# antoyang/FrozenBiLM

Hardware: AMD Instinct MI355X
Metric: video-text samples/sec (MLM fwd+bwd) DeBERTa-XL+adapters (higher is better)
Workload: dtype bf16; 1 GPU; DeBERTa-v2-XLarge(24L)+adapters ds8/8, B=32/GPU, T=10x1024, L=256 (S=266), MLM fwd+bwd+allreduce+clip+Adam, dropout 0.1 live, seeded random weights; global_batch=32, seq_len=266, parallelism=dp1, dead_layer23_encoder_pass=skipped (output unused, SURVEY fact 6); FLOPs still counted

## Files before the change

### frozenbilm_amd/csrc/attn_fwd.hip

```cpp
#include "attn_common.h"
#include "../../include/fbl.h"

namespace {
using namespace attn;

struct AttnArgs {
  const bf16* q; const bf16* k; const bf16* v; const bf16* pk; const bf16* pq;
  long ldq, ldk, ldp;
  long ldv;
  const int16_t* relidx;
  const int32_t* mask;
  const int32_t* klen;
  const int32_t* border;
  float scale, p_drop;
  uint64_t seed; const uint64_t* seed_dev;
  bf16* ctx;
  long ldo;
  float* lse;
  int B, S, Sp, nh, span2;
  int lin;
  int dbg;
  const int32_t* row0;
  bf16* psave;
  float* msave;
};
#ifdef FBL_DEBUG_SWITCHES
#define ATTN_DBG(bit) (a.dbg & (bit))
#else
#define ATTN_DBG(bit) 0
#endif

constexpr int LTW = 100;
constexpr int SM_KS = 0;
constexpr int SM_VS = SM_KS + 8192;
constexpr int SM_T1 = SM_VS + 8192;
constexpr int SM_T2 = SM_T1 + 64 * LTW * 2;
constexpr int SM_KM = SM_T2 + 64 * LTW * 2;
constexpr int SM_QS = SM_KM + 256;
constexpr int SM_IDX = SM_QS + 8192;
__host__ __device__ constexpr int sm_total(int Sp) { return SM_IDX + 2 * Sp * 2; }

struct TileRegs {
  bf16x8 k[2], v[2];
  int km;
};

template <int OCC, bool PF, bool PACKED = false, bool SAVEP = false>
__global__ __launch_bounds__(256, OCC) void attn_fwd_kernel(AttnArgs a) {
  extern __shared__ __attribute__((aligned(16))) char smem[];
  const int tid = threadIdx.x, lane = tid & 63;
  const int w = __builtin_amdgcn_readfirstlane(tid >> 6);
  const int c = lane & 15, g = lane >> 4;
  const int S = a.S, Sp = a.Sp;
  const WgCoord wc = wg_coord((S + 63) / 64, a.nh, a.B, a.border);
  const int i0 = wc.x * 64, h = wc.h, b = wc.b;
  const int i = i0 + w * 16 + c;
  const int ic = min(i, S - 1);

  int16_t* idx = (int16_t*)(smem + SM_IDX);
  float* kms = (float*)(smem + SM_KM);
  f16* T1 = (f16*)(smem + SM_T1);
  f16* T2 = (f16*)(smem + SM_T2);

  const int kl = a.klen ? min(a.klen[b], S) : S;
  const int nkt = (i0 < kl) ? (kl + 63) / 64 : 0;
  const long rb = PACKED ? (long)a.row0[b] : (long)b * S;
  const int lim = PACKED ? min(a.row0[b + 1] - a.row0[b], S) : S;
  if (nkt > 0) load_idx_padded(idx, a.relidx, S, Sp, tid, 256);

  const bool qvalid = i < S && a.mask[(long)b * S + ic] != 0;

  float m_run = -INFINITY, l_run = 0.f;
  f32x4 o[4];
#pragma unroll
  for (int dt = 0; dt < 4; ++dt) o[dt] = (f32x4){0.f, 0.f, 0.f, 0.f};

  const DropKey dk = attn_drop_key(a.p_drop > 0.f ? fbl_seed(a.seed, a.seed_dev) : 0, b * a.nh + h, a.p_drop);
  const float k2 = a.scale * LOG2E;
  const int tq = Sp - 1;
  const int izero = a.relidx[S - 1];
  const bf16* pkh = a.pk + h * 64 + g * 8;
  const bf16* pqh = a.pq + h * 64 + g * 8;
  const int my_t0 = (0x5243 >> (w * 4)) & 15, my_t1 = (0x1670 >> (w * 4)) & 15;

  const int srow = tid >> 3, sch = tid & 7;
  const int fb0 = c * 128 + ((g ^ (c & 7)) << 4), fb1 = fb0 ^ 64;
  const int sb = srow * 128 + ((sch ^ (srow & 7)) << 4);
  auto load_tile = [&](int jt, TileRegs& R) {
    const int j0 = jt * 64;
#pragma unroll
    for (int t = 0; t < 2; ++t) {
      const int row = srow + t * 32;
      const int j = min(j0 + row, lim - 1);
      R.k[t] = *(const bf16x8*)(a.k + (rb + j) * a.ldk + h * 64 + sch * 8);
      R.v[t] = *(const bf16x8*)(a.v + (rb + j) * a.ldv + h * 64 + sch * 8);
    }
    R.km = a.mask[(long)b * S + min(j0 + lane, S - 1)];
  };
  auto store_tile = [&](const TileRegs& R, int j0) {
#pragma unroll
    for (int t = 0; t < 2; ++t) {
      *(bf16x8*)(smem + SM_KS + sb + t * 4096) = R.k[t];
      *(bf16x8*)(smem + SM_VS + sb + t * 4096) = R.v[t];
    }
    if (tid < 64) kms[tid] = (j0 + tid < S && R.km != 0) ? 1.f : 0.f;
  };

  TileRegs R;
  if (PF && nkt > 0) load_tile(0, R);
  if (nkt > 0) {
#pragma unroll
    for (int t = 0; t < 2; ++t) {
      const int row = srow + t * 32;
      *(bf16x8*)(smem + SM_QS + sb + t * 4096) = *(const bf16x8*)(a.q + (rb + min(i0 + row, lim - 1)) * a.ldq + h * 64 + sch * 8);
    }
    __syncthreads();
  }
  for (int jt = 0; jt < nkt; ++jt) {
    const int j0 = jt * 64;
    const bool band = !ATTN_DBG(32) && max(abs(i0 - (j0 + 63)), abs(i0 + 63 - j0)) < a.lin;
    int r_lo, t0q[4], t0k[4];
    if (band) {
      r_lo = izero + i0 - (j0 + 63);
#pragma unroll
      for (int x = 0; x < 4; ++x) { t0q[x] = x; t0k[x] = 3 - x; }
    } else {
      r_lo = __builtin_amdgcn_readfirstlane((int)idx[i0 - (j0 + 63) + tq]);
#pragma unroll
      for (int x = 0; x < 4; ++x) {
        t0q[x] = (__builtin_amdgcn_readfirstlane((int)idx[i0 + x * 16 - (j0 + 63) + tq]) - r_lo) >> 4;
        t0k[x] = (__builtin_amdgcn_readfirstlane((int)idx[i0 - (j0 + x * 16 + 15) + tq]) - r_lo) >> 4;
      }
    }
    const int ntile = band ? 5 : 6;
    bf16x8 apk[2][2], apq[2][2];
    if (!ATTN_DBG(2)) {
#pragma unroll
      for (int u = 0; u < 2; ++u) {
        const long ro = (long)min(r_lo + (u ? my_t1 : my_t0) * 16 + c, a.span2 - 1) * a.ldp;
        apk[u][0] = *(const bf16x8*)(pkh + ro);
        apk[u][1] = *(const bf16x8*)(pkh + ro + 32);
        apq[u][0] = *(const bf16x8*)(pqh + ro);
        apq[u][1] = *(const bf16x8*)(pqh + ro + 32);
      }
    }
    if (!PF) load_tile(jt, R);
    store_tile(R, j0);
    __syncthreads();

    f32x4 sacc[4];
    const bf16x8 qf[2] = {*(const bf16x8*)(smem + SM_QS + w * 2048 + fb0), *(const bf16x8*)(smem + SM_QS + w * 2048 + fb1)};
#pragma unroll
    for (int nt = 0; nt < 4; ++nt) {
      f32x4 acc = (f32x4){0.f, 0.f, 0.f, 0.f};
      acc = __builtin_amdgcn_mfma_f32_16x16x32_bf16(*(const bf16x8*)(smem + SM_KS + nt * 2048 + fb0), qf[0], acc, 0, 0, 0);
      acc = __builtin_amdgcn_mfma_f32_16x16x32_bf16(*(const bf16x8*)(smem + SM_KS + nt * 2048 + fb1), qf[1], acc, 0, 0, 0);
      sacc[nt] = acc;
    }
    if (!ATTN_DBG(2)) {
      const f16 ninf = (f16)(-INFINITY);
      f16* t1s = T1 + c * LTW + g * 4;
      f16* t2s = T2 + c * LTW + g * 4;
      auto pair1 = [&](const bf16x8& a0, const bf16x8& a1, int x, int rel) {
        f32x4 acc = (f32x4){0.f, 0.f, 0.f, 0.f};
        acc = __builtin_amdgcn_mfma_f32_16x16x32_bf16(a0, *(const bf16x8*)(smem + SM_QS + x * 2048 + fb0), acc, 0, 0, 0);
        acc = __builtin_amdgcn_mfma_f32_16x16x32_bf16(a1, *(const bf16x8*)(smem + SM_QS + x * 2048 + fb1), acc, 0, 0, 0);
        *(f16x4*)(t1s + x * 16 * LTW + rel * 16) = to_f16x4(acc);
      };
      auto pair2 = [&](const bf16x8& a0, const bf16x8& a1, int x, int rel) {
        f32x4 acc = (f32x4){0.f, 0.f, 0.f, 0.f};
        acc = __builtin_amdgcn_mfma_f32_16x16x32_bf16(a0, *(const bf16x8*)(smem + SM_KS + x * 2048 + fb0), acc, 0, 0, 0);
        acc = __builtin_amdgcn_mfma_f32_16x16x32_bf16(a1, *(const bf16x8*)(smem + SM_KS + x * 2048 + fb1), acc, 0, 0, 0);
        const f16x4 tv = to_f16x4(acc);
        *(f16x4*)(t2s + x * 16 * LTW + rel * 16) = kms[x * 16 + c] != 0.f ? tv : (f16x4){ninf, ninf, ninf, ninf};
      };
      {
#pragma unroll
        for (int u = 0; u < 2; ++u) {
          const int t = u ? my_t1 : my_t0;
#pragma unroll
          for (int x = 0; x < 4; ++x) {
            const int rel1 = t - t0q[x];
            if (rel1 >= 0 && rel1 < ntile) pair1(apk[u][0], apk[u][1], x, rel1);
            const int rel2 = t - t0k[x];
            if (rel2 >= 0 && rel2 < ntile) pair2(apq[u][0], apq[u][1], x, rel2);
          }
        }
      }
    }
    __syncthreads();
    if (PF) load_tile(min(jt + 1, nkt - 1), R);

    float p[16];
    float mx = -INFINITY;
    if (ATTN_DBG(1)) {
#pragma unroll
      for (int e = 0; e < 16; ++e) { p[e] = sacc[e >> 2][e & 3]; mx = fmaxf(mx, p[e]); }
    } else if (band) {
      const f16* t1p = T1 + (w * 16 + c) * LTW + c + 63 - g * 4;
      const f16* t2p = T2 + g * 4 * LTW + w * 16 + c + 15 - g * 4;
#pragma unroll
      for (int nt = 0; nt < 4; ++nt)
#pragma unroll
        for (int r = 0; r < 4; ++r) {
          const float s = sacc[nt][r] + (float)t1p[-(nt * 16 + r)] + (float)t2p[(nt * 16 + r) * LTW - r];
          p[nt * 4 + r] = s;
          mx = fmaxf(mx, s);
        }
    } else {
      const int16_t* ib = idx + (i - j0 - g * 4 + tq - 63);
      int sbw = r_lo;
#pragma unroll
      for (int x = 0; x < 4; ++x) sbw = (w == x) ? r_lo + 16 * t0q[x] : sbw;
      const f16* t1row = T1 + (w * 16 + c) * LTW - sbw;
      const f16* t2g = T2 + g * 4 * LTW - r_lo;
#pragma unroll
      for (int nt = 0; nt < 4; ++nt) {
        const f16* t2n = t2g - 16 * t0k[nt];
#pragma unroll
        for (int r = 0; r < 4; ++r) {
          const int wi = ib[63 - nt * 16 - r];
          const float s = sacc[nt][r] + (float)t1row[wi] + (float)t2n[(nt * 16 + r) * LTW + wi];
          p[nt * 4 + r] = s;
          mx = fmaxf(mx, s);
        }
      }
    }
    mx = fmaxf(mx, __shfl_xor(mx, 16, 64));
    mx = fmaxf(mx, __shfl_xor(mx, 32, 64));
    const float m_new = fmaxf(m_run, mx);
    float alpha = 1.f, psum = 0.f;
    if (!(m_new > -INFINITY)) {
#pragma unroll
      for (int e = 0; e < 16; ++e) p[e] = 0.f;
    } else {
      alpha = __builtin_amdgcn_exp2f((m_run - m_new) * k2);
      const float mk = -m_new * k2;
#pragma unroll
      for (int e = 0; e < 16; ++e) {
        p[e] = __builtin_amdgcn_exp2f(fmaf(p[e], k2, mk));
        psum += p[e];
      }
    }
    psum += __shfl_xor(psum, 16, 64);
    psum += __shfl_xor(psum, 32, 64);
    l_run = l_run * alpha + psum;
    m_run = m_new;
#pragma unroll
    for (int dt = 0; dt < 4; ++dt) o[dt] *= alpha;
    float kf[16];
#pragma unroll
    for (int e = 0; e < 16; ++e) kf[e] = 1.f;
    if (a.p_drop > 0.f && !ATTN_DBG(8)) {
#pragma unroll
      for (int nt = 0; nt < 4; ++nt)
#pragma unroll
        for (int bb = 0; bb < 2; ++bb) {
          uint32_t x, y;
          attn_drop_block(dk, i >> 1, (j0 + nt * 16 + g * 4 + bb * 2) >> 1, Sp >> 1, &x, &y);
          kf[nt * 4 + bb * 2] = attn_drop_keep(dk, x, y, i & 1, 0);
          kf[nt * 4 + bb * 2 + 1] = attn_drop_keep(dk, x, y, i & 1, 1);
        }
    }
    if constexpr (SAVEP) {
      bf16* pp = a.psave + (((long)b * a.nh + h) * Sp + i) * Sp + j0 + g * 4;
#pragma unroll
      for (int nt = 0; nt < 4; ++nt) {
        bf16x4 v4;
#pragma unroll
        for (int r = 0; r < 4; ++r) v4[r] = f2bf(kf[nt * 4 + r] == 0.f ? -p[nt * 4 + r] : p[nt * 4 + r]);
        *(bf16x4*)(pp + nt * 16) = v4;
      }
      if (g == 0 && i < S) a.msave[(((long)b * a.nh + h) * (Sp >> 6) + jt) * S + i] = m_new * k2;
    }
#pragma unroll
    for (int e = 0; e < 16; ++e) p[e] *= kf[e];
    if (!ATTN_DBG(4))
#pragma unroll
    for (int kk = 0; kk < 2; ++kk) {
      bf16x8 pf;
#pragma unroll
      for (int e = 0; e < 4; ++e) {
        pf[e] = f2bf(p[(2 * kk) * 4 + e]);
        pf[4 + e] = f2bf(p[(2 * kk + 1) * 4 + e]);
      }
#pragma unroll
      for (int dt = 0; dt < 4; ++dt) {
        const int r = g * 4 + (c >> 2);
        const int ch = dt * 2 + ((c >> 1) & 1), sub = (c & 1) * 8;
        const char* vb = smem + SM_VS + r * 128 + ((ch ^ (r & 7)) << 4) + sub;
        union { tr16x4 h[2]; bf16x8 v; } u;
        u.h[0] = lds_tr16((const bf16*)(vb + kk * 4096));
        u.h[1] = lds_tr16((const bf16*)(vb + kk * 4096 + 2048));
        o[dt] = __builtin_amdgcn_mfma_f32_16x16x32_bf16(u.v, pf, o[dt], 0, 0, 0);
      }
    }
    __syncthreads();
  }

  const float inv_l = (qvalid && l_run > 0.f) ? 1.f / l_run : 0.f;
  if (i < S) {
    if (i < lim) {
      bf16* op = a.ctx + (rb + i) * a.ldo + h * 64 + g * 4;
#pragma unroll
      for (int dt = 0; dt < 4; ++dt) {
        f32x4 v = o[dt] * inv_l;
        if (inv_l == 0.f) v = (f32x4){0.f, 0.f, 0.f, 0.f};
        *(bf16x4*)(op + dt * 16) = (bf16x4){f2bf(v[0]), f2bf(v[1]), f2bf(v[2]), f2bf(v[3])};
      }
    }
    if (g == 0 && a.lse)
      a.lse[((long)b * a.nh + h) * S + i] = (qvalid && l_run > 0.f) ? m_run * a.scale + __logf(l_run) : INFINITY;
  }
}

__global__ __launch_bounds__(128) void attn_probs_kernel(const bf16* q, const bf16* k, long ldq, const bf16* pk, const bf16* pq,
                                                         long ldp, const int16_t* relidx, const int32_t* mask, const float* lse,
                                                         float scale, float* probs, int B, int S, int nh) {
  __shared__ float qs[64];
  const int i = blockIdx.x % S, h = (blockIdx.x / S) % nh, b = blockIdx.x / (S * nh);
  const long row = (long)b * S + i;
  if (threadIdx.x < 64) qs[threadIdx.x] = bf2f(q[row * ldq + h * 64 + threadIdx.x]);
  __syncthreads();
  const bool qvalid = mask[row] != 0;
  const float l = lse[((long)b * nh + h) * S + i];
  float* out = probs + (((long)b * nh + h) * S + i) * S;
  for (int j = threadIdx.x; j < S; j += blockDim.x) {
    float p = 0.f;
    if (qvalid && mask[(long)b * S + j] != 0) {
      const int r = relidx[i - j + S - 1];
      const bf16* kj = k + ((long)b * S + j) * ldq + h * 64;
      const bf16* pkr = pk + (long)r * ldp + h * 64;
      const bf16* pqr = pq + (long)r * ldp + h * 64;
      float s = 0.f;
#pragma unroll 8
      for (int d = 0; d < 64; ++d) {
        const float kd = bf2f(kj[d]);
        s += qs[d] * (kd + bf2f(pkr[d])) + kd * bf2f(pqr[d]);
      }
      p = __expf(s * scale - l);
    }
    out[j] = p;
  }
}

}

extern "C" int fbl_disent_attn_probs(const void* q, const void* k, int64_t ldq, const void* pk, const void* pq, int64_t ldp,
                                     const int16_t* relidx, const int32_t* mask, const float* lse, float scale,
                                     float* probs, int B, int S, int nh, void* stream) {
  if (S < 1 || S > 512) return FBL_ERR_SHAPE;
  if (!q || !k || !pk || !pq || !relidx || !mask || !lse || !probs) return FBL_ERR_ARG;
  if (B <= 0 || nh <= 0) return 0;
  hipLaunchKernelGGL(attn_probs_kernel, dim3((unsigned)(B * nh * S)), dim3(128), 0, (hipStream_t)stream, (const bf16*)q,
                     (const bf16*)k, (long)ldq, (const bf16*)pk, (const bf16*)pq, (long)ldp, relidx, mask, lse, scale, probs, B, S,
                     nh);
  FBL_CHECK_LAUNCH();
  return 0;
}

extern "C" int fbl_disent_attn_fwd(const void* q, int64_t ldq, const void* k, int64_t ldk, const void* v, int64_t ldv,
                                   const void* pk, const void* pq, int64_t ldp,
                                   const int16_t* relidx, const int32_t* mask, const int32_t* klen,
                                   const int32_t* border, float scale, float p_drop, uint64_t seed,
                                   const uint64_t* seed_dev, void* ctx, int64_t ldo, float* lse, int B, int S, int Sp, int nh, int span2,
                                   int lin_span, const int32_t* row0, void* psave, float* msave, void* stream) {
  if (S < 1 || S > 512 || Sp < S || Sp % 64) return FBL_ERR_SHAPE;
  if ((ldq % 8) || (ldk % 8) || (ldv % 8) || (ldp % 8) || (ldo % 4)) return FBL_ERR_ALIGN;
  if (lin_span < 0 || 2 * lin_span > span2) return FBL_ERR_ARG;
  if (row0 && !klen) return FBL_ERR_ARG;
  if ((psave != nullptr) != (msave != nullptr) || (psave && !lse)) return FBL_ERR_ARG;
  if (B <= 0 || nh <= 0) return 0;
  AttnArgs a{(const bf16*)q, (const bf16*)k, (const bf16*)v, (const bf16*)pk, (const bf16*)pq, ldq, ldk, ldp, ldv, relidx, mask, klen, border, scale, p_drop, seed, seed_dev, (bf16*)ctx, ldo, lse, B, S, Sp, nh, span2, lin_span, 0, row0,
             (bf16*)psave, msave};
  static const int dbg = FBL_ENV_INT("FBL_ATTN_DBG", 0);
  a.dbg = dbg;
  attn_debug_init();
  const int smem_bytes = sm_total(Sp);
  static int attr_bytes = 0;
  if (smem_bytes > attr_bytes) {
    const void* fns[] = {(const void*)attn_fwd_kernel<3, true>, (const void*)attn_fwd_kernel<3, true, true>,
                         (const void*)attn_fwd_kernel<3, true, false, true>, (const void*)attn_fwd_kernel<3, true, true, true>,
#ifdef FBL_DEBUG_SWITCHES
                         (const void*)attn_fwd_kernel<3, false>, (const void*)attn_fwd_kernel<3, false, true>,
                         (const void*)attn_fwd_kernel<3, false, false, true>, (const void*)attn_fwd_kernel<3, false, true, true>,
#endif
    };
    for (const void* fn : fns) {
      hipError_t e = hipFuncSetAttribute(fn, hipFuncAttributeMaxDynamicSharedMemorySize, smem_bytes);
      if (e != hipSuccess) return (int)e;
    }
    attr_bytes = smem_bytes;
  }
  dim3 grid((unsigned)((S + 63) / 64) * nh * B);
#define FBL_FWD_LAUNCH(PF_)                                                                                             \
  do {                                                                                                                  \
    if (row0 && psave)                                                                                                  \
      hipLaunchKernelGGL((attn_fwd_kernel<3, PF_, true, true>), grid, dim3(256), smem_bytes, (hipStream_t)stream, a);   \
    else if (row0)                                                                                                      \
      hipLaunchKernelGGL((attn_fwd_kernel<3, PF_, true>), grid, dim3(256), smem_bytes, (hipStream_t)stream, a);         \
    else if (psave)                                                                                                     \
      hipLaunchKernelGGL((attn_fwd_kernel<3, PF_, false, true>), grid, dim3(256), smem_bytes, (hipStream_t)stream, a);  \
    else                                                                                                                \
      hipLaunchKernelGGL((attn_fwd_kernel<3, PF_>), grid, dim3(256), smem_bytes, (hipStream_t)stream, a);               \
  } while (0)
#ifdef FBL_DEBUG_SWITCHES
  static const int pf = FBL_ENV_INT("FBL_ATTN_PF", 1);
  if (!pf) FBL_FWD_LAUNCH(false);
  else
#endif
    FBL_FWD_LAUNCH(true);
#undef FBL_FWD_LAUNCH
  FBL_CHECK_LAUNCH();
  return 0;
}
```

Before: 787.9 samples/s.

## Use buffer loads and prefetch position fragments one tile ahead in attention forward

Global loads for Q, K, V, positional K/Q, mask and relidx in the disentangled attention forward kernel now go through buffer resource descriptors with 32-bit offsets instead of 64-bit pointer arithmetic. The apk/apq positional fragments for the next key tile are issued right after the next K/V tile prefetch, so their latency overlaps the current tile's softmax and PV work. The prologue loads of relidx, Q and the first fragments are hoisted ahead of the LDS stores, and workgroups with no key tiles now exit early. Host checks reject leading dimensions that would overflow the 32-bit buffer offsets, and register pressure rises from holding the prefetched fragments.

```diff
diff --git a/frozenbilm_amd/csrc/attn_fwd.hip b/frozenbilm_amd/csrc/attn_fwd.hip
--- a/frozenbilm_amd/csrc/attn_fwd.hip
+++ b/frozenbilm_amd/csrc/attn_fwd.hip
@@ -45,6 +45,17 @@
   int km;
 };
 
+typedef __attribute__((ext_vector_type(2))) unsigned int u32x2;
+__device__ __forceinline__ int buf_ld4(__amdgpu_buffer_rsrc_t r, uint32_t voff, uint32_t soff) {
+  return (int)__builtin_amdgcn_raw_buffer_load_b32(r, voff, soff, 0);
+}
+__device__ __forceinline__ int16_t buf_ld2(__amdgpu_buffer_rsrc_t r, uint32_t voff, uint32_t soff) {
+  return (int16_t)__builtin_amdgcn_raw_buffer_load_b16(r, voff, soff, 0);
+}
+__device__ __forceinline__ void buf_st8(__amdgpu_buffer_rsrc_t r, uint32_t voff, uint32_t soff, bf16x4 v) {
+  __builtin_amdgcn_raw_buffer_store_b64(__builtin_bit_cast(u32x2, v), r, voff, soff, 0);
+}
+
 template <int OCC, bool PF, bool PACKED = false, bool SAVEP = false>
 __global__ __launch_bounds__(256, OCC) void attn_fwd_kernel(AttnArgs a) {
   extern __shared__ __attribute__((aligned(16))) char smem[];
@@ -66,36 +77,40 @@
   const int nkt = (i0 < kl) ? (kl + 63) / 64 : 0;
   const long rb = PACKED ? (long)a.row0[b] : (long)b * S;
   const int lim = PACKED ? min(a.row0[b + 1] - a.row0[b], S) : S;
-  if (nkt > 0) load_idx_padded(idx, a.relidx, S, Sp, tid, 256);
-
-  const bool qvalid = i < S && a.mask[(long)b * S + ic] != 0;
-
-  float m_run = -INFINITY, l_run = 0.f;
-  f32x4 o[4];
-#pragma unroll
-  for (int dt = 0; dt < 4; ++dt) o[dt] = (f32x4){0.f, 0.f, 0.f, 0.f};
-
-  const DropKey dk = attn_drop_key(a.p_drop > 0.f ? fbl_seed(a.seed, a.seed_dev) : 0, b * a.nh + h, a.p_drop);
+  if (nkt == 0) {
+    if (i < S) {
+      if (i < lim) {
+        bf16* op = a.ctx + (rb + i) * a.ldo + h * 64 + g * 4;
+#pragma unroll
+        for (int dt = 0; dt < 4; ++dt) *(bf16x4*)(op + dt * 16) = (bf16x4){f2bf(0.f), f2bf(0.f), f2bf(0.f), f2bf(0.f)};
+      }
+      if (g == 0 && a.lse) a.lse[((long)b * a.nh + h) * S + i] = INFINITY;
+    }
+    return;
+  }
+
   const float k2 = a.scale * LOG2E;
   const int tq = Sp - 1;
-  const int izero = a.relidx[S - 1];
-  const bf16* pkh = a.pk + h * 64 + g * 8;
-  const bf16* pqh = a.pq + h * 64 + g * 8;
   const int my_t0 = (0x5243 >> (w * 4)) & 15, my_t1 = (0x1670 >> (w * 4)) & 15;
 
   const int srow = tid >> 3, sch = tid & 7;
   const int fb0 = c * 128 + ((g ^ (c & 7)) << 4), fb1 = fb0 ^ 64;
   const int sb = srow * 128 + ((sch ^ (srow & 7)) << 4);
+
+  const __amdgpu_buffer_rsrc_t rq = buf_rsrc(a.q + rb * a.ldq + h * 64), rk = buf_rsrc(a.k + rb * a.ldk + h * 64),
+                               rv = buf_rsrc(a.v + rb * a.ldv + h * 64), rpk = buf_rsrc(a.pk + h * 64),
+                               rpq = buf_rsrc(a.pq + h * 64), rmask = buf_rsrc(a.mask + (long)b * S),
+                               ridx = buf_rsrc(a.relidx);
+  const uint32_t ldq2 = (uint32_t)a.ldq * 2, ldk2 = (uint32_t)a.ldk * 2, ldv2 = (uint32_t)a.ldv * 2, ldp2 = (uint32_t)a.ldp * 2;
   auto load_tile = [&](int jt, TileRegs& R) {
     const int j0 = jt * 64;
 #pragma unroll
     for (int t = 0; t < 2; ++t) {
-      const int row = srow + t * 32;
-      const int j = min(j0 + row, lim - 1);
-      R.k[t] = *(const bf16x8*)(a.k + (rb + j) * a.ldk + h * 64 + sch * 8);
-      R.v[t] = *(const bf16x8*)(a.v + (rb + j) * a.ldv + h * 64 + sch * 8);
-    }
-    R.km = a.mask[(long)b * S + min(j0 + lane, S - 1)];
+      const uint32_t j = (uint32_t)min(j0 + srow + t * 32, lim - 1);
+      R.k[t] = buf_ld16(rk, j * ldk2 + sch * 16, 0);
+      R.v[t] = buf_ld16(rv, j * ldv2 + sch * 16, 0);
+    }
+    R.km = buf_ld4(rmask, (uint32_t)min(j0 + lane, S - 1) * 4, 0);
   };
   auto store_tile = [&](const TileRegs& R, int j0) {
 #pragma unroll
@@ -105,27 +120,62 @@
     }
     if (tid < 64) kms[tid] = (j0 + tid < S && R.km != 0) ? 1.f : 0.f;
   };
-
+  auto in_band = [&](int j0) { return !ATTN_DBG(32) && max(abs(i0 - (j0 + 63)), abs(i0 + 63 - j0)) < a.lin; };
+  bf16x8 apk[2][2], apq[2][2];
+  auto load_frags = [&](int r_lo) {
+#pragma unroll
+    for (int u = 0; u < 2; ++u) {
+      const uint32_t ro = (uint32_t)clampi(r_lo + (u ? my_t1 : my_t0) * 16 + c, 0, a.span2 - 1) * ldp2 + g * 16;
+      apk[u][0] = buf_ld16(rpk, ro, 0);
+      apk[u][1] = buf_ld16(rpk, ro + 64, 0);
+      apq[u][0] = buf_ld16(rpq, ro, 0);
+      apq[u][1] = buf_ld16(rpq, ro + 64, 0);
+    }
+  };
+
+  const int16_t e0 = buf_ld2(ridx, 0, (uint32_t)(in_band(0) ? S - 1 : clampi(i0 - 63 + S - 1, 0, 2 * S - 2)) * 2);
+  int16_t ie[4];
+#pragma unroll
+  for (int u = 0; u < 4; ++u) ie[u] = buf_ld2(ridx, (uint32_t)clampi(tid + u * 256 - (Sp - S), 0, 2 * S - 2) * 2, 0);
+  bf16x8 qr[2];
+#pragma unroll
+  for (int t = 0; t < 2; ++t) qr[t] = buf_ld16(rq, (uint32_t)min(i0 + srow + t * 32, lim - 1) * ldq2 + sch * 16, 0);
   TileRegs R;
-  if (PF && nkt > 0) load_tile(0, R);
-  if (nkt > 0) {
-#pragma unroll
-    for (int t = 0; t < 2; ++t) {
-      const int row = srow + t * 32;
-      *(bf16x8*)(smem + SM_QS + sb + t * 4096) = *(const bf16x8*)(a.q + (rb + min(i0 + row, lim - 1)) * a.ldq + h * 64 + sch * 8);
-    }
+  if (PF) load_tile(0, R);
+  const int qm = buf_ld4(rmask, (uint32_t)ic * 4, 0);
+  const DropKey dk = attn_drop_key(a.p_drop > 0.f ? fbl_seed(a.seed, a.seed_dev) : 0, b * a.nh + h, a.p_drop);
+  int r_lo = __builtin_amdgcn_readfirstlane((int)e0);
+  if (in_band(0)) r_lo += i0 - 63;
+  if (!ATTN_DBG(2)) load_frags(r_lo);
+  __builtin_amdgcn_sched_barrier(0);
+#pragma unroll
+  for (int u = 0; u < 4; ++u) idx[min(tid + u * 256, 2 * Sp - 1)] = ie[u];
+#pragma unroll
+  for (int t = 0; t < 2; ++t) *(bf16x8*)(smem + SM_QS + sb + t * 4096) = qr[t];
+
+  float m_run = -INFINITY, l_run = 0.f;
+  f32x4 o[4];
+#pragma unroll
+  for (int dt = 0; dt < 4; ++dt) o[dt] = (f32x4){0.f, 0.f, 0.f, 0.f};
+  __amdgpu_buffer_rsrc_t rps;
+  uint32_t pso = 0;
+  if constexpr (SAVEP) {
+    rps = buf_rsrc(a.psave + ((long)b * a.nh + h) * Sp * Sp);
+    pso = ((uint32_t)i * Sp + g * 4) * 2;
+  }
+
+  int jt = 0;
+  do {
+    const int j0 = jt * 64;
+    const bool band = in_band(j0);
+    if (!PF) load_tile(jt, R);
+    store_tile(R, j0);
     __syncthreads();
-  }
-  for (int jt = 0; jt < nkt; ++jt) {
-    const int j0 = jt * 64;
-    const bool band = !ATTN_DBG(32) && max(abs(i0 - (j0 + 63)), abs(i0 + 63 - j0)) < a.lin;
-    int r_lo, t0q[4], t0k[4];
+    int t0q[4], t0k[4];
     if (band) {
-      r_lo = izero + i0 - (j0 + 63);
 #pragma unroll
       for (int x = 0; x < 4; ++x) { t0q[x] = x; t0k[x] = 3 - x; }
     } else {
-      r_lo = __builtin_amdgcn_readfirstlane((int)idx[i0 - (j0 + 63) + tq]);
 #pragma unroll
       for (int x = 0; x < 4; ++x) {
         t0q[x] = (__builtin_amdgcn_readfirstlane((int)idx[i0 + x * 16 - (j0 + 63) + tq]) - r_lo) >> 4;
@@ -133,20 +183,7 @@
       }
     }
     const int ntile = band ? 5 : 6;
-    bf16x8 apk[2][2], apq[2][2];
-    if (!ATTN_DBG(2)) {
-#pragma unroll
-      for (int u = 0; u < 2; ++u) {
-        const long ro = (long)min(r_lo + (u ? my_t1 : my_t0) * 16 + c, a.span2 - 1) * a.ldp;
-        apk[u][0] = *(const bf16x8*)(pkh + ro);
-        apk[u][1] = *(const bf16x8*)(pkh + ro + 32);
-        apq[u][0] = *(const bf16x8*)(pqh + ro);
-        apq[u][1] = *(const bf16x8*)(pqh + ro + 32);
-      }
-    }
-    if (!PF) load_tile(jt, R);
-    store_tile(R, j0);
-    __syncthreads();
+    const int r_cur = r_lo;
 
     f32x4 sacc[4];
     const bf16x8 qf[2] = {*(const bf16x8*)(smem + SM_QS + w * 2048 + fb0), *(const bf16x8*)(smem + SM_QS + w * 2048 + fb1)};
@@ -189,7 +226,14 @@
       }
     }
     __syncthreads();
-    if (PF) load_tile(min(jt + 1, nkt - 1), R);
+    const int jn = min(jt + 1, nkt - 1);
+    if (PF) load_tile(jn, R);
+    {
+      const int izero = __builtin_amdgcn_readfirstlane((int)idx[Sp - 1]);
+      const int r_tab = __builtin_amdgcn_readfirstlane((int)idx[i0 - (jn * 64 + 63) + tq]);
+      r_lo = in_band(jn * 64) ? izero + i0 - (jn * 64 + 63) : r_tab;
+      if (!ATTN_DBG(2)) load_frags(r_lo);
+    }
 
     float p[16];
     float mx = -INFINITY;
@@ -209,11 +253,11 @@
         }
     } else {
       const int16_t* ib = idx + (i - j0 - g * 4 + tq - 63);
-      int sbw = r_lo;
-#pragma unroll
-      for (int x = 0; x < 4; ++x) sbw = (w == x) ? r_lo + 16 * t0q[x] : sbw;
+      int sbw = r_cur;
+#pragma unroll
+      for (int x = 0; x < 4; ++x) sbw = (w == x) ? r_cur + 16 * t0q[x] : sbw;
       const f16* t1row = T1 + (w * 16 + c) * LTW - sbw;
-      const f16* t2g = T2 + g * 4 * LTW - r_lo;
+      const f16* t2g = T2 + g * 4 * LTW - r_cur;
 #pragma unroll
       for (int nt = 0; nt < 4; ++nt) {
         const f16* t2n = t2g - 16 * t0k[nt];
@@ -263,13 +307,12 @@
         }
     }
     if constexpr (SAVEP) {
-      bf16* pp = a.psave + (((long)b * a.nh + h) * Sp + i) * Sp + j0 + g * 4;
 #pragma unroll
       for (int nt = 0; nt < 4; ++nt) {
         bf16x4 v4;
 #pragma unroll
         for (int r = 0; r < 4; ++r) v4[r] = f2bf(kf[nt * 4 + r] == 0.f ? -p[nt * 4 + r] : p[nt * 4 + r]);
-        *(bf16x4*)(pp + nt * 16) = v4;
+        buf_st8(rps, pso + nt * 32, (uint32_t)j0 * 2, v4);
       }
       if (g == 0 && i < S) a.msave[(((long)b * a.nh + h) * (Sp >> 6) + jt) * S + i] = m_new * k2;
     }
@@ -296,8 +339,9 @@
       }
     }
     __syncthreads();
-  }
-
+  } while (++jt < nkt);
+
+  const bool qvalid = i < S && qm != 0;
   const float inv_l = (qvalid && l_run > 0.f) ? 1.f / l_run : 0.f;
   if (i < S) {
     if (i < lim) {
@@ -367,6 +411,9 @@
                                    int lin_span, const int32_t* row0, void* psave, float* msave, void* stream) {
   if (S < 1 || S > 512 || Sp < S || Sp % 64) return FBL_ERR_SHAPE;
   if ((ldq % 8) || (ldk % 8) || (ldv % 8) || (ldp % 8) || (ldo % 4)) return FBL_ERR_ALIGN;
+  for (const int64_t ld : {ldq, ldk, ldv})
+    if (ld < 0 || (uint64_t)ld * 2u * (uint64_t)S >= (1ull << 32)) return FBL_ERR_SHAPE;
+  if (ldp < 0 || span2 < 1 || (uint64_t)ldp * 2u * (uint64_t)span2 >= (1ull << 32)) return FBL_ERR_SHAPE;
   if (lin_span < 0 || 2 * lin_span > span2) return FBL_ERR_ARG;
   if (row0 && !klen) return FBL_ERR_ARG;
   if ((psave != nullptr) != (msave != nullptr) || (psave && !lse)) return FBL_ERR_ARG;
```

Measured after the change: 787.0 samples/s. Within noise of the previous version (-0.1%).
